# cvlab-stonybrook/s-volsdf

Measured on AMD Instinct MI355X. Metric: rendered rays/sec (1024-ray batch, 128 samples), higher is better.
Workload: dtype f32 (every product, forward and backward, as three fp16 MFMA products of two-piece fp16 operands with f32 accumulate; activation blocks hold both pieces: float32 accuracy class); 1 GPU; configs[1]: VolOpt.train_step (forward + MVS prior lookup + loss + backward + clip/guard/Adam), train mode, fast=1: 1024 rays/GPU x 128 coarse + 98 composited samples + 2048 eikonal points, 8x256 SDF MLP + 4x256 radiance MLP; mode=train, mlp_precision=fp16x2, launch=eager launches, rays_per_gpu=1024, rays_total=1024

## Files before the change

### s-volsdf_amd/csrc/svs_mlp_bwd.hip

```cpp
#include "svs_mlp_dev.h"
#include "svs_mlp_bwd_args.h"
#include "svs_ticket.h"

namespace svs {
namespace mlp {


__global__ __launch_bounds__(kThreads, 1) void rgb_bwd_kernel(RgbBwdArgs a) {
  extern __shared__ __attribute__((aligned(16))) unsigned char smem[];
  Stream st;
  st.g = a.stream; st.buf = reinterpret_cast<f32x4*>(smem); st.cur = 1;
  const int lane = threadIdx.x & 63, half = lane >> 5, wave = threadIdx.x >> 6;
  const int wtile = blockIdx.x * kWaves + wave;
  const int p = wtile * kTilePts + (lane & 31);
  const bool livep = p < a.P;
  const int pc = livep ? p : a.P - 1;
  const size_t LS = block_stride();
  const float* rb = a.rbuf + (size_t)wtile * kBlockF;
  float* zb = a.zbuf + (size_t)wtile * kBlockF;

  st.prefetch<kW4TF4>();
  float dz[3];
#pragma unroll
  for (int c = 0; c < 3; ++c) {
// ... 277 lines not shown
    for (int d = 16; d >= 1; d >>= 1) bsum += __shfl_xor(bsum, d);
    if (lane == 0) atomicAdd(&out[256], bsum);
  }
  det::pass_turn(ticket, blockIdx.x);
}

struct UnpackArgs {
  const float* dWk;
  const float* dbk;
  int ldw;
  int map;
  int rows, cols, row_off;
  const float* v; const float* g;
  float* grad_v; float* grad_g; float* grad_b;
  const float* row0;
};

__device__ __forceinline__ int kernel_col(int map, int c) {
  if (map == 1) return c < 217 ? c : (c < 249 ? 224 + (c - 217) : 217 + (c - 249));
  if (map == 2) return c < 15 ? 256 + c : c - 15;
  if (map == 3) {
    if (c < 172) return c;
    const int e = c - 172;
    return e < 32 ? 224 + e : (e < 64 ? 192 + (e - 32) : 172 + (e - 64));
  }
  if (map == 4) return c < 27 ? 256 + c : c - 27;
  return c;
}

__device__ __forceinline__ void unpack_row(const UnpackArgs& a, int o, int lane) {
  if (o >= a.rows) return;
  const float fac = (a.map == 1 || a.map == 3) ? 0.70710678118654752f : 1.0f;
  const bool is_row0 = a.row0 && o == 0;
  const int ko = o - a.row_off;
  auto dweff = [&](int c) -> float {
    if (is_row0) return a.row0[c];
    return a.dWk[(size_t)ko * a.ldw + kernel_col(a.map, c)] * fac;
  };
  if (lane == 0 && a.grad_b) a.grad_b[o] = is_row0 ? a.row0[256] : (a.dbk ? a.dbk[ko] : 0.0f);
  if (!a.g) {
    for (int c = lane; c < a.cols; c += 64) a.grad_v[(size_t)o * a.cols + c] = dweff(c);
    return;
  }
  double nn = 0.0, dot = 0.0;
  for (int c = lane; c < a.cols; c += 64) {
    const double vv = (double)a.v[(size_t)o * a.cols + c];
    nn += vv * vv; dot += vv * (double)dweff(c);
  }
  for (int d = 32; d >= 1; d >>= 1) { nn += __shfl_xor(nn, d); dot += __shfl_xor(dot, d); }
  const double nrm = __builtin_sqrt(nn);
  const float gg = a.g[o];
  const float k1 = (float)((double)gg / nrm), k2 = (float)((double)gg * dot / (nrm * nn));
  if (lane == 0) a.grad_g[o] = (float)(dot / nrm);
  for (int c = lane; c < a.cols; c += 64)
    a.grad_v[(size_t)o * a.cols + c] = k1 * dweff(c) - k2 * a.v[(size_t)o * a.cols + c];
}

__global__ __launch_bounds__(256) void unpack_wgrad_kernel(UnpackArgs a) {
  unpack_row(a, blockIdx.x * 4 + (threadIdx.x >> 6), threadIdx.x & 63);
}

constexpr int kMaxUnpackJobs = 24;
struct UnpackMulti {
  UnpackArgs job[kMaxUnpackJobs];
  int first_block[kMaxUnpackJobs + 1];
  int n;
};
__global__ __launch_bounds__(256) void unpack_wgrad_multi_kernel(UnpackMulti m) {
  int j = 0;
  while (j + 1 < m.n && (int)blockIdx.x >= m.first_block[j + 1]) ++j;
  unpack_row(m.job[j], ((int)blockIdx.x - m.first_block[j]) * 4 + (threadIdx.x >> 6), threadIdx.x & 63);
}

}
}

using namespace svs;
using namespace svs::mlp;

namespace {
int tiles_of(int n_points) { return (n_points + kWgPts - 1) / kWgPts * kWaves; }
template <typename K>
int set_lds_b(K kernel, int bytes, const char* who) {
  hipError_t e = hipFuncSetAttribute(reinterpret_cast<const void*>(kernel), hipFuncAttributeMaxDynamicSharedMemorySize, bytes);
  if (e != hipSuccess) { set_error("%s: hipFuncSetAttribute: %s", who, hipGetErrorString(e)); return (int)e; }
  return SVS_OK;
}
}

struct svs_unpack_job {
  const float *dWk, *dbk;
  int ldw, map, rows, cols, row_off;
  const float *weight_v, *weight_g, *row0;
  float *grad_v, *grad_g, *grad_b;
};

extern "C" {

size_t svs_block_bytes(int n_points, int blocks_per_tile) {
  return (size_t)tiles_of(n_points) * blocks_per_tile * (kBlockF + 64) * sizeof(float);
}
size_t svs_rgb_zbuf_bytes(int n_points) { return svs_block_bytes(n_points, 5); }
size_t svs_sdf_ubuf_bytes(int n_points) { return svs_block_bytes(n_points, 9); }
size_t svs_sdf_gbuf_bytes(int n_points) { return svs_block_bytes(n_points, 8); }

int svs_rgb_bwd(int n_points, const float* d_rgb, const float* rgb, const float* rbuf, const float* stream, int precision,
                float* zbuf, float* feat_bar, float* d_normals, float* absmax, void* hip_stream) {
  if (!d_rgb || !rgb || !rbuf || !stream || !zbuf || !feat_bar || !d_normals || n_points <= 0) {
    set_error("svs_rgb_bwd: null/invalid argument"); return SVS_EINVAL;
  }
  RgbBwdArgs a{n_points, d_rgb, rgb, rbuf, reinterpret_cast<const f32x4*>(stream), zbuf, feat_bar, d_normals, absmax};
  if (is_h2(precision)) {
    if (!absmax) { set_error("svs_rgb_bwd: fp16x2 needs absmax"); return SVS_EINVAL; }
    return launch_rgb_bwd_h2(a, precision == kFmtF16x2, (hipStream_t)hip_stream);
  }
  if (precision != kFmtF32) { set_error("svs_rgb_bwd: unknown precision %d", precision); return SVS_EINVAL; }
  static int once = set_lds_b(rgb_bwd_kernel, kLdsBytes, "svs_rgb_bwd");
  if (once) return once;
  rgb_bwd_kernel<<<(n_points + kWgPts - 1) / kWgPts, kThreads, kLdsBytes, (hipStream_t)hip_stream>>>(a);
  return check_launch("svs_rgb_bwd");
}

int svs_sdf_bwd_a(const float* points, int n_points, const float* cam, int cam_stride, const float* dirs, const float* z,
                  int S, int n_rays, const float* d_grad, const unsigned char* clamp_mask, const float* hbuf,
                  const float* gbuf, const float* stream, int precision, float* ubuf, float* a2buf, float* pebuf,
                  float* absmax, void* hip_stream) {
  SdfBwdAArgs a;
  const bool h2 = is_h2(precision);
  if (n_points < 0 || n_rays < 0 || (n_points == 0 && n_rays == 0) || (n_points > 0 && !points) ||
      (n_rays > 0 && !(cam && dirs && z && S > 0)) || !d_grad || !hbuf || (!h2 && !gbuf) || !stream || !ubuf || (!h2 && !a2buf) ||
      !pebuf) {
    set_error("svs_sdf_bwd_a: null/invalid argument"); return SVS_EINVAL;
  }
  a.src.pts = points; a.src.cam = cam; a.src.dirs = dirs; a.src.z = z; a.src.cam_stride = cam_stride;
  a.src.S = S > 0 ? S : 1; a.src.n_ray = n_rays * (S > 0 ? S : 0); a.src.P = a.src.n_ray + n_points;
  a.d_grad = d_grad; a.clamp_mask = clamp_mask; a.hbuf = hbuf; a.gbuf = gbuf;
  a.stream = reinterpret_cast<const f32x4*>(stream); a.ubuf = ubuf; a.a2buf = a2buf; a.pebuf = pebuf;
  a.absmax = absmax;
  if (h2) {
    if (!absmax) { set_error("svs_sdf_bwd_a: fp16x2 needs absmax"); return SVS_EINVAL; }
    return launch_sdf_bwd_a_h2(a, precision == kFmtF16x2, (hipStream_t)hip_stream);
  }
  if (precision != kFmtF32) { set_error("svs_sdf_bwd_a: unknown precision %d", precision); return SVS_EINVAL; }
  static int once = set_lds_b(sdf_bwd_a_kernel, kLdsBytes, "svs_sdf_bwd_a");
  if (once) return once;
  sdf_bwd_a_kernel<<<(a.src.P + kWgPts - 1) / kWgPts, kThreads, kLdsBytes, (hipStream_t)hip_stream>>>(a);
  return check_launch("svs_sdf_bwd_a");
}

int svs_sdf_bwd_b(int n_points, const float* d_sdf, const unsigned char* clamp_mask, const float* feat_bar,
                  int n_feat_points, const float* hbuf, const float* gbuf, const float* a2buf, const float* ubuf,
                  const float* stream, int precision, float* abuf, float* sbar_out, float* absmax, void* hip_stream) {
  const bool h2 = is_h2(precision);
  if (!hbuf || !gbuf || (h2 ? !ubuf : !a2buf) || !stream || !abuf || !sbar_out || n_points <= 0 || n_feat_points % 32) {
    set_error("svs_sdf_bwd_b: null/invalid argument (n_feat_points must be a multiple of 32)"); return SVS_EINVAL;
  }
  SdfBwdBArgs a{n_points, d_sdf, clamp_mask, feat_bar, n_feat_points / 32, hbuf, gbuf, a2buf, ubuf,
                reinterpret_cast<const f32x4*>(stream) + kSdfTrainPassBF4, abuf, sbar_out, absmax,
                gbuf + 7 * (size_t)tiles_of(n_points) * kBlockF, (size_t)kBlockF};
  if (h2) {
    if (!absmax) { set_error("svs_sdf_bwd_b: fp16x2 needs absmax"); return SVS_EINVAL; }
    return launch_sdf_bwd_b_h2(a, precision == kFmtF16x2, (hipStream_t)hip_stream);
  }
  if (precision != kFmtF32) { set_error("svs_sdf_bwd_b: unknown precision %d", precision); return SVS_EINVAL; }
  static int once = set_lds_b(sdf_bwd_b_kernel, kLdsBytes, "svs_sdf_bwd_b");
  if (once) return once;
  sdf_bwd_b_kernel<<<(n_points + kWgPts - 1) / kWgPts, kThreads, kLdsBytes, (hipStream_t)hip_stream>>>(a);
  return check_launch("svs_sdf_bwd_b");
}

int svs_lin8_row0_grad(const float* hbuf, const float* ubuf, const float* sbar, int n_points, int precision, float* out257,
                       void* hip_stream) {
  if (!hbuf || !sbar || !out257 || n_points <= 0) { set_error("svs_lin8_row0_grad: bad argument"); return SVS_EINVAL; }
  if (is_h2(precision)) return launch_lin8_row0_h2(hbuf, ubuf, sbar, n_points, tiles_of(n_points), out257, precision == kFmtF16x2, (hipStream_t)hip_stream);
  if (precision != kFmtF32) { set_error("svs_lin8_row0_grad: unknown precision %d", precision); return SVS_EINVAL; }
  const int n_tiles = (n_points + 31) / 32;
  const int grid = n_tiles < 1024 ? n_tiles : 1024;
  const det::Ticket ticket{det::take_slots(1), 0u, (unsigned)grid};
  lin8_row0_kernel<<<grid, 256, 0, (hipStream_t)hip_stream>>>(hbuf, ubuf, sbar, n_tiles, tiles_of(n_points), n_points, out257, ticket);
  return check_launch("svs_lin8_row0_grad");
}

int svs_unpack_wgrad(const float* dWk, const float* dbk, int ldw, int map, int rows, int cols, int row_off,
                     const float* weight_v, const float* weight_g, const float* row0, float* grad_v, float* grad_g,
                     float* grad_b, void* hip_stream) {
  if (!dWk || !weight_v || !grad_v || rows < 1 || cols < 1 || map < 0 || map > 4 || (weight_g && !grad_g)) {
    set_error("svs_unpack_wgrad: bad argument"); return SVS_EINVAL;
  }
  UnpackArgs a{dWk, dbk, ldw, map, rows, cols, row_off, weight_v, weight_g, grad_v, grad_g, grad_b, row0};
  unpack_wgrad_kernel<<<(rows + 3) / 4, 256, 0, (hipStream_t)hip_stream>>>(a);
  return check_launch("svs_unpack_wgrad");
}

int svs_unpack_wgrad_multi(const svs_unpack_job* jobs, int n_jobs, void* hip_stream) {
  if (!jobs || n_jobs < 1 || n_jobs > kMaxUnpackJobs) { set_error("svs_unpack_wgrad_multi: 1..%d jobs", kMaxUnpackJobs); return SVS_EINVAL; }
  UnpackMulti m;
  m.n = n_jobs;
  int blocks = 0;
  for (int i = 0; i < n_jobs; ++i) {
    const svs_unpack_job& q = jobs[i];
    if (!q.dWk || !q.weight_v || !q.grad_v || q.rows < 1 || q.cols < 1 || q.map < 0 || q.map > 4 || (q.weight_g && !q.grad_g)) {
      set_error("svs_unpack_wgrad_multi: bad job %d", i); return SVS_EINVAL;
    }
    m.job[i] = UnpackArgs{q.dWk, q.dbk, q.ldw, q.map, q.rows, q.cols, q.row_off, q.weight_v, q.weight_g, q.grad_v, q.grad_g, q.grad_b, q.row0};
    m.first_block[i] = blocks;
    blocks += (q.rows + 3) / 4;
  }
  m.first_block[n_jobs] = blocks;
  unpack_wgrad_multi_kernel<<<blocks, 256, 0, (hipStream_t)hip_stream>>>(m);
  return check_launch("svs_unpack_wgrad_multi");
}

}
```

### s-volsdf_amd/csrc/svs_mlp_bwd_h2.hip

```cpp
#include "svs_mlp_h2_dev.h"
#include "svs_mlp_host.h"
#include "svs_mlp_bwd_args.h"
#include "svs_mlp_h2_trunk.h"
#include "svs_mlp_bwd_h2_dev.h"
#include "svs_ticket.h"
#include <cstdlib>

namespace svs {
namespace mlp {

template <bool GP>
struct RgbBwdEpi {
  f32x16 prev;
  TilePieces r;
  float v8[8];
  Pieces2* out;
  float* zblk;
  PointScale* ps;
  int lane;
  __device__ __forceinline__ void b(int tp, int rr) {
    float v = prev[rr] * ps->inv_in;
    v = hi_at(r, rr) > 0.0f ? v : 0.0f;
    pin(v);
    ps->track(v);
    v8[rr & 7] = v * ps->s_out;
    if ((rr & 7) == 7) {
      split8(v8, out->h[2 * tp + (rr >> 3)], out->m[2 * tp + (rr >> 3)]);
      pin(out->h[2 * tp + (rr >> 3)], out->m[2 * tp + (rr >> 3)]);
    }
    if (rr == 9) store_piece(zblk, 2 * tp, lane, out->h[2 * tp], 0);
    if (GP && rr == 11) store_piece(zblk, 2 * tp, lane, out->m[2 * tp], 1);
    if (rr == 15) store_grad<GP>(zblk, 2 * tp + 1, lane, out->h[2 * tp + 1], out->m[2 * tp + 1]);
  }
  __device__ __forceinline__ void all(int tp) {
#pragma unroll
    for (int rr = 0; rr < 16; ++rr) b(tp, rr);
  }
};

template <bool GP>
__device__ __forceinline__ void rgb_bwd_layer_h2(Stream& st, const Pieces2& in, Pieces2& out, const float* rblk, float* zblk,
                                                 float* zrec, PointScale& ps, int lane) {
  RgbBwdEpi<GP> ep;
  ep.out = &out; ep.zblk = zblk; ep.ps = &ps; ep.lane = lane;
  store_record(zrec, lane, ps.s_out, 0.0f);
  TilePieces rnext;
  load_tile_hi(rblk, 0, lane, rnext);
#pragma unroll
  for (int t = 0; t < 8; ++t) {
    const TilePieces rcur = rnext;
    auto rload = [&](int s) {
      if (t == 7) return;
      if (s == 10) rnext.h[0] = load_piece(rblk, 2 * (t + 1), lane);
      if (s == 12) rnext.h[1] = load_piece(rblk, 2 * (t + 1) + 1, lane);
    };
    f32x16 acc;
    if (t == 0) acc = tile_mma_h2_pf<16, kChunkF4>(st, in, lane, NoEpi(), NoEpi(), rload);
    else acc = tile_mma_h2_pf<16, kChunkF4>(st, in, lane, NoEpi(), [&](int s) { ep.b(t - 1, s); }, rload);
    ep.prev = acc; ep.r = rcur;
    constexpr int kSt = GP ? 4 : 2;
    if (t == 0) st.advance_keep<2>();
    else if (t < 7) st.advance_keep<2 + kSt>();
    else st.advance_keep<kSt>();
  }
  ep.all(7);
  ps.next();
}

template <bool GP>
__global__ __launch_bounds__(kThreads, 1) void rgb_bwd_h2_kernel(RgbBwdArgs a) {
  extern __shared__ __attribute__((aligned(16))) unsigned char smem[];
  Stream st;
  st.g = a.stream; st.buf = reinterpret_cast<f32x4*>(smem); st.cur = 1;
  const int lane = threadIdx.x & 63, half = lane >> 5, wave = threadIdx.x >> 6;
  const int wtile = blockIdx.x * kWaves + wave;
  const int p = wtile * kTilePts + (lane & 31);
  const bool livep = p < a.P;
  const int pc = livep ? p : a.P - 1;
  const size_t LS = block_stride();
  const float* rb = a.rbuf + (size_t)wtile * kBlockF;
  float* zb = a.zbuf + (size_t)wtile * kBlockF;
  const size_t T = (size_t)gridDim.x * kWaves;
  auto zrec = [&](int l) { return record_ptr(a.zbuf, 5, T, l, wtile); };

  st.prefetch<kW4TF4>();
  float dz[3];
  float m0 = 0.0f;
#pragma unroll
  for (int c = 0; c < 3; ++c) {
    const float o = a.rgb[3 * pc + c];
    dz[c] = (livep && half == 0) ? a.d_rgb[3 * pc + c] * o * (1.0f - o) : 0.0f;
    m0 = __builtin_fmaxf(m0, __builtin_fabsf(dz[c]));
  }
  m0 = __builtin_fmaxf(m0, __shfl_xor(m0, 32));
  PointScale ps;
  ps.start(m0, 0.0f);
  {
    float v8[8] = {dz[0] * ps.s_in, dz[1] * ps.s_in, dz[2] * ps.s_in, 0.0f, 0.0f, 0.0f, 0.0f, 0.0f};
    store_grad8<GP>(zb + 4 * LS, 0, lane, v8);
    store_record(zrec(4), lane, ps.s_in, m0);
  }
  st.advance();
  Pieces2 pa, pb;
  st.prefetch<kChunkF4>();
  {
    const f32x4* c = st.cur_buf();
    const float* r4 = rb + 3 * LS;
    float* z3 = zb + 3 * LS;
    store_record(zrec(3), lane, ps.s_out, 0.0f);
#pragma unroll
    for (int t = 0; t < 8; ++t) {
      TilePieces r;
      load_tile_hi(r4, t, lane, r);
      const f32x4 w = c[t * 64 + lane];
      f32x16 acc = (f32x16)(0.0f);
      acc = __builtin_amdgcn_mfma_f32_32x32x2f32(w[0], dz[0], acc, 0, 0, 0);
      acc = __builtin_amdgcn_mfma_f32_32x32x2f32(w[1], dz[1], acc, 0, 0, 0);
      acc = __builtin_amdgcn_mfma_f32_32x32x2f32(w[2], dz[2], acc, 0, 0, 0);
#pragma unroll
      for (int i = 0; i < 16; ++i) { acc[i] = hi_at(r, i) > 0.0f ? acc[i] : 0.0f; ps.track(acc[i]); }
      split_tile_scaled(acc, t, pa, ps.s_out);
      store_grad<GP>(z3, 2 * t, lane, pa.h[2 * t], pa.m[2 * t]);
      store_grad<GP>(z3, 2 * t + 1, lane, pa.h[2 * t + 1], pa.m[2 * t + 1]);
    }
  }
  ps.next();
  st.advance();
  rgb_bwd_layer_h2<GP>(st, pa, pb, rb + 2 * LS, zb + 2 * LS, zrec(2), ps, lane);
  rgb_bwd_layer_h2<GP>(st, pb, pa, rb + 1 * LS, zb + 1 * LS, zrec(1), ps, lane);
  rgb_bwd_layer_h2<GP>(st, pa, pb, rb, zb, zrec(0), ps, lane);
  float* fb = a.feat_bar + (size_t)wtile * kBlockF;
  float fmax = 0.0f;
  const float s_f = ps.s_out;
  {
    f32x16 prev;
    float v8[8];
    auto slice = [&](int tp, int r) {
      const float v = prev[r] * ps.inv_in;
      fmax = __builtin_fmaxf(fmax, __builtin_fabsf(v));
      v8[r & 7] = v * s_f;
      if ((r & 7) == 7) store_grad8<GP>(fb, 2 * tp + (r >> 3), lane, v8);
    };
#pragma unroll
    for (int t = 0; t < 9; ++t) {
      if (t < 8) st.prefetch<kChunkF4>();
      f32x16 acc;
      if (t == 0) acc = tile_mma_h2<16>(st.cur_buf(), pb, lane);
      else acc = tile_mma_h2<16>(st.cur_buf(), pb, lane, NoEpi(), [&](int s) { slice(t - 1, s); });
      if (t < 8) { prev = acc; st.advance(); }
      else if (half == 1 && livep) {
        a.d_normals[3 * p] = acc[4] * ps.inv_in; a.d_normals[3 * p + 1] = acc[5] * ps.inv_in;
        a.d_normals[3 * p + 2] = acc[6] * ps.inv_in;
      }
    }
  }
  fmax = __builtin_fmaxf(fmax, __shfl_xor(fmax, 32));
  store_record(record_ptr(a.feat_bar, 1, T, 0, wtile), lane, s_f, fmax);
  publish_max(a.absmax + 1, ps.gmax);
  publish_max(a.absmax + 2, fmax);
}

constexpr int kSpliceF = 20;

template <bool SPLIT, bool GP>
struct PassAEpi {
  f32x16 prev;
  TilePieces h;
  float v, s1;
  float v8[8];
  f16x8 up[2], uq[2];
  Pieces2* out;
  float* ublk;
  float* urec;
  PointScale* ps;
  const float* splice;
  float vm;
  int lane, half;
  bool l3;

  __device__ __forceinline__ void begin() {
    if (lane < 32) urec[lane] = ps->s_out;
    vm = 0.0f;
  }
  __device__ __forceinline__ void end() {
    vm = __builtin_fmaxf(vm, __shfl_xor(vm, 32));
    if (lane >= 32) urec[lane] = vm;
  }
  __device__ __forceinline__ void a(int r) {
    v = prev[r] * ps->inv_in;
    s1 = 1.0f - __builtin_amdgcn_exp2f(grad_times<GP>(h, r, -100.0f * 1.44269504088896341f));
    pin(v); pin(s1);
  }
  template <bool LATE = false>
  __device__ __forceinline__ void b(int tp, int r) {
    float u = v * s1;
    float w = __builtin_fabsf(v) * (100.0f - 100.0f * s1);
    if (tp == 6 && r >= 12 && l3) {
      const bool sp = half == 1 || r >= 13;
      const float us = splice[(16 + (r - 12)) * kThreads];
      u = sp ? us : u;
      w = sp ? 0.0f : w;
    }
    pin(u); pin(w);
    emit<LATE>(tp, r, u, w);
  }
  template <bool LATE = false>
  __device__ __forceinline__ void emit(int tp, int r, float u, float w) {
    vm = __builtin_fmaxf(vm, w);
    ps->track(u);
    v8[r & 7] = u * ps->s_out;
    if ((r & 7) == 7) {
      const int k = 2 * tp + (r >> 3), q = r >> 3;
      if (SPLIT) {
        split8(v8, out->h[k], out->m[k]);
        pin(out->h[k], out->m[k]);
        up[q] = out->h[k];
        if (GP) uq[q] = out->m[k];
      } else if (GP) {
        split8(v8, up[q], uq[q]);
      } else {
        up[q] = hi8(v8, 1.0f);
      }
      if (!LATE) store_grad<GP>(ublk, k, lane, up[q], uq[q]);
    }
  }
  __device__ __forceinline__ void store_slot(int tp, int s) {
    if (s == 9) store_piece(ublk, 2 * tp, lane, up[0], 0);
    if (GP && s == 11) store_piece(ublk, 2 * tp, lane, uq[0], 1);
    if (s == 15) store_grad<GP>(ublk, 2 * tp + 1, lane, up[1], uq[1]);
  }
  __device__ __forceinline__ void all(int tp) {
#pragma unroll
    for (int r = 0; r < 16; ++r) { a(r); b(tp, r); }
  }
  __device__ __forceinline__ void splice_tile7() {
#pragma unroll
    for (int r = 0; r < 16; ++r) emit(7, r, splice[r * kThreads], 0.0f);
  }
};

template <bool SPLIT, bool LAST, bool GP>
__device__ __forceinline__ void pass_a_layer_h2(Stream& st, const Pieces2& in, PassAEpi<SPLIT, GP>& ep, const float* hblk, int lane) {
  ep.begin();
#pragma unroll
  for (int t = 0; t < 8; ++t) {
    if (t == 7 && ep.l3) break;
    TilePieces hload;
    load_tile_grad<GP>(hblk, t, lane, hload);
    const bool fetch = !(LAST && t == 7);
    f32x16 acc;
    if (!fetch) acc = tile_mma_h2<16>(st.cur_buf(), in, lane, [&](int s) { ep.a(s); }, [&](int s) { ep.b(t - 1, s); });
    else if (t == 0) acc = tile_mma_h2_pf<16, kChunkF4>(st, in, lane, NoEpi(), NoEpi());
    else acc = tile_mma_h2_pf<16, kChunkF4>(st, in, lane, [&](int s) { ep.a(s); },
                                            [&](int s) { ep.template b<true>(t - 1, s); ep.store_slot(t - 1, s); });
    ep.prev = acc; ep.h = hload;
    if (fetch) {
      if (t == 0) st.advance();
      else st.advance_keep<GP ? 4 : 2>();
    }
  }
  if (ep.l3) { ep.all(6); ep.splice_tile7(); }
  else ep.all(7);
  ep.end();
  ep.ps->next();
}

template <bool GP>
__global__ __launch_bounds__(kThreads, 1) void sdf_bwd_a_h2_kernel(SdfBwdAArgs a) {
  extern __shared__ __attribute__((aligned(16))) unsigned char smem[];
  Stream st;
  st.g = a.stream; st.buf = reinterpret_cast<f32x4*>(smem); st.cur = 1;
  float* splice = reinterpret_cast<float*>(smem + kLdsBytes) + threadIdx.x;
  const int lane = threadIdx.x & 63, half = lane >> 5, wave = threadIdx.x >> 6;
  const int wtile = blockIdx.x * kWaves + wave;
  const int p = wtile * kTilePts + (lane & 31);
  const int pc = p < a.src.P ? p : a.src.P - 1;

  st.prefetch<kChunk0F4>();
  PointScale ps;
  Pieces2 pa, pb;
  const size_t LS = block_stride();
  const float* hb = a.hbuf + (size_t)wtile * kBlockF;
  float* ub = a.ubuf + (size_t)wtile * kBlockF;
  const size_t T = (size_t)gridDim.x * kWaves;
  auto urec = [&](int l) { return record_ptr(a.ubuf, 9, T, l, wtile); };
  {
    float x0, x1, x2;
    load_point(a.src, p, x0, x1, x2);
    PosEnc pe;
    pe.compute(x0, x1, x2);
    float nb[3] = {a.d_grad[3 * pc], a.d_grad[3 * pc + 1], a.d_grad[3 * pc + 2]};
    if (p >= a.src.P || (a.clamp_mask && a.clamp_mask[pc])) { nb[0] = nb[1] = nb[2] = 0.0f; }
    PosEnc u0;
    float m0 = 0.0f;
#pragma unroll
    for (int q = 0; q < 40; ++q) {
      float coef = 1.0f; int c = q;
      if (q >= 3 && q < kPeDim) {
        const int f = (q - 3) / 6, w = (q - 3) % 6;
        const float sc = (float)(1 << f);
        c = w < 3 ? w : w - 3;
        coef = w < 3 ? sc * pe.v[q + 3] : -sc * pe.v[q - 3];
      }
// ... 365 lines not shown
```

### s-volsdf_amd/csrc/svs_mlp_h2.hip

```cpp
#include "svs_mlp_h2_dev.h"
#include "svs_mlp_host.h"
#include "svs_mlp_args.h"
#include "svs_mlp_h2_trunk.h"
#include "svs_blocks_h2.h"

namespace svs {
namespace mlp {

__global__ __launch_bounds__(kThreads, 1) void sdf_only_h2_kernel(SdfOnlyArgs a) {
  extern __shared__ __attribute__((aligned(16))) unsigned char smem[];
  if (a.gate && a.gate[(size_t)(blockIdx.x * kWgPts / a.gate_points) * a.gate_stride] == 0) return;
  Stream st;
  st.g = a.stream;
  st.buf = reinterpret_cast<f32x4*>(smem);
  st.cur = 1;
  const int lane = threadIdx.x & 63, half = lane >> 5, wave = threadIdx.x >> 6;
  const int p = (blockIdx.x * kWaves + wave) * kTilePts + (lane & 31);

  st.prefetch<kChunk0F4>();
  float x0, x1, x2;
  load_point(a.src, p, x0, x1, x2);
  const float r2 = x0 * x0 + x1 * x1 + x2 * x2;
  PosEnc pe;
  pe.compute(x0, x1, x2);
// ... 160 lines not shown
        store_grad<GP>(gb + 7 * block_stride(), 2 * t + 1, lane, xn.h[2 * t + 1], xn.m[2 * t + 1]);
      }
    }
    if (GBUF) store_record(grec0 + 7 * rec_stride, lane, 1.0f, __builtin_fmaxf(gm7, __shfl_xor(gm7, 32)));
    st.advance();
  }
  float* ft = a.feat_tiles ? a.feat_tiles + (size_t)wtile * kBlockF : nullptr;
  {
    f32x16 prev;
    float v8[8];
    f16x8 fh[2], fm[2];
    auto slice = [&](int tp, int r) {
      v8[r & 7] = prev[r];
      if ((r & 7) == 7) { split8(v8, fh[r >> 3], fm[r >> 3]); pin(fh[r >> 3], fm[r >> 3]); }
      if (!ft) return;
      if (r == 9) store_piece(ft, 2 * tp, lane, fh[0], 0);
      if (r == 11) store_piece(ft, 2 * tp, lane, fm[0], 1);
      if (r == 15) { store_piece(ft, 2 * tp + 1, lane, fh[1], 0); store_piece(ft, 2 * tp + 1, lane, fm[1], 1); }
    };
#pragma unroll
    for (int t = 0; t < 8; ++t) {
      f32x16 acc;
      if (t == 0) acc = tile_mma_h2_pf<16, kChunkF4>(st, x, lane, NoEpi(), NoEpi());
      else acc = tile_mma_h2_pf<16, kChunkF4>(st, x, lane, NoEpi(), [&](int s) { slice(t - 1, s); });
      prev = acc;
      if (ft && t > 0) st.advance_keep<4>();
      else st.advance();
    }
#pragma unroll
    for (int r = 0; r < 16; ++r) slice(7, r);
  }
  f32x16 skip7 = (f32x16)(0.0f);
  f32x16 skip6 = (f32x16)(0.0f);
  for (int l = 7; l >= 1; l -= 2) {
    reverse_layer_h2<GBUF, GP>(st, xn, x, l, hb, gb, grec0, rec_stride, skip6, skip7, lane, half);
    if (l > 1) reverse_layer_h2<GBUF, GP>(st, x, xn, l - 1, hb, gb, grec0, rec_stride, skip6, skip7, lane, half);
  }
  st.prefetch<kChunkF4>();
  f32x16 gpe0 = tile_mma_h2<16>(st.cur_buf(), x, lane);
  st.advance();
  f32x16 gpe1 = tile_mma_h2<16>(st.cur_buf(), x, lane);
  gpe0 += skip7;
  gpe1 += skip6;

  if (!GBUF) {
    int p2 = p;
    asm volatile("" : "+v"(p2));
    load_point(a.src, p2, x0, x1, x2);
    pe.compute(x0, x1, x2);
  }
  float dx0 = 0.0f, dx1 = 0.0f, dx2 = 0.0f;
  auto accum = [&](int q, float g, bool active) {
    if (q < 0 || q >= kPeDim) return;
    float coef = 1.0f;
    int c = q;
    if (q >= 3) {
      const int f = (q - 3) / 6, w = (q - 3) % 6;
      const float sc = (float)(1 << f);
      c = w < 3 ? w : w - 3;
      coef = w < 3 ? sc * pe.v[q + 3] : -sc * pe.v[q - 3];
    }
    const float term = active ? coef * g : 0.0f;
    if (c == 0) dx0 += term; else if (c == 1) dx1 += term; else dx2 += term;
  };
#pragma unroll
  for (int r = 0; r < 16; ++r) {
    accum(rho(r), gpe0[r], half == 0);
    accum(rho(r) + 4, gpe0[r], half == 1);
    accum(rho(r) >= 25 ? 32 + rho(r) - 25 : -1, gpe1[r], half == 0);
    accum(rho(r) + 4 >= 25 ? 32 + rho(r) + 4 - 25 : -1, gpe1[r], half == 1);
  }
  dx0 += __shfl_xor(dx0, 32); dx1 += __shfl_xor(dx1, 32); dx2 += __shfl_xor(dx2, 32);

  bool clamped = false;
  if (a.sphere_radius > 0.0f && p < a.clamp_n) {
    const float nrm = __builtin_sqrtf(x0 * x0 + x1 * x1 + x2 * x2);
    const float sphere = a.sphere_scale * (a.sphere_radius - nrm);
    if (sphere < sdf) {
      sdf = sphere;
      const float k = -a.sphere_scale / nrm;
      dx0 = k * x0; dx1 = k * x1; dx2 = k * x2;
      clamped = true;
    }
  }
  if (half == 0 && p < a.src.P && a.clamp_mask) a.clamp_mask[p] = clamped ? 1 : 0;
  if (half == 0 && p < a.src.P) {
    a.sdf[p] = sdf;
    a.grad[3 * p + 0] = dx0; a.grad[3 * p + 1] = dx1; a.grad[3 * p + 2] = dx2;
  }
}

template <bool GP>
struct RgbEpi {
  f32x16 prev;
  float v8[8];
  Pieces2* out;
  float* rblk;
  int lane;
  __device__ __forceinline__ void b(int tp, int r) {
    float v;
    asm("v_max_f32 %0, 0, %1" : "=v"(v) : "v"(prev[r]));
    pin(v);
    v8[r & 7] = v;
    if ((r & 7) == 7) {
      split8(v8, out->h[2 * tp + (r >> 3)], out->m[2 * tp + (r >> 3)]);
      pin(out->h[2 * tp + (r >> 3)], out->m[2 * tp + (r >> 3)]);
    }
    if (rblk) {
      if (r == 11) store_piece(rblk, 2 * tp, lane, out->h[2 * tp], 0);
      if (GP && r == 13) store_piece(rblk, 2 * tp, lane, out->m[2 * tp], 1);
      if (r == 15) store_grad<GP>(rblk, 2 * tp + 1, lane, out->h[2 * tp + 1], out->m[2 * tp + 1]);
    }
  }
  __device__ __forceinline__ void all(int tp) {
#pragma unroll
    for (int r = 0; r < 16; ++r) b(tp, r);
  }
};

template <int KS, int N16NEXT_LAST, bool GP>
__device__ __forceinline__ void rgb_layer_h2(RgbStream& st, const Pieces2& in, Pieces2& out, float* rblk, int lane) {
  RgbEpi<GP> ep;
  ep.out = &out; ep.rblk = rblk; ep.lane = lane;
  constexpr int kNext = KS == 17 ? kRgbChunk0F4 : kChunkF4;
#pragma unroll
  for (int t = 0; t < 8; ++t) {
    auto relu = [&](int s) { if (s < 16) ep.b(t - 1, s); };
    f32x16 acc;
    if (t == 0) acc = tile_mma_h2_pf<KS, kNext>(st, in, lane, NoEpi(), NoEpi());
    else if (t < 7) acc = tile_mma_h2_pf<KS, kNext>(st, in, lane, NoEpi(), relu);
    else acc = tile_mma_h2_pf<KS, N16NEXT_LAST>(st, in, lane, NoEpi(), relu);
    ep.prev = acc;
    if (rblk && t > 0) st.template advance_keep<GP ? 4 : 2>();
    else st.advance();
  }
  ep.all(7);
}

template <bool GP>
__global__ __launch_bounds__(kThreads, 1) void rgb_h2_kernel(RgbArgs a) {
  extern __shared__ __attribute__((aligned(16))) unsigned char smem[];
  RgbStream st;
  st.g = a.stream; st.buf = reinterpret_cast<f32x4*>(smem); st.cur = 1;
  const int lane = threadIdx.x & 63, half = lane >> 5, wave = threadIdx.x >> 6;
  const int wtile = blockIdx.x * kWaves + wave;
  const int p = wtile * kTilePts + (lane & 31);
  const int pc = p < a.src.P ? p : a.src.P - 1;

  st.prefetch<kRgbChunk0F4>();
  float x0, x1, x2;
  load_point(a.src, p, x0, x1, x2);
  const float* vd = a.view + 3 * (size_t)(a.view_S > 0 ? pc / a.view_S : pc);
  const float d0 = vd[0], d1 = vd[1], d2 = vd[2];
  float ex[16];
  ex[0] = x0; ex[1] = x1; ex[2] = x2; ex[3] = d0; ex[4] = d1; ex[5] = d2;
  ex[6] = sinf(d0); ex[7] = sinf(d1); ex[8] = sinf(d2); ex[9] = cosf(d0); ex[10] = cosf(d1); ex[11] = cosf(d2);
  ex[12] = a.normals[3 * pc]; ex[13] = a.normals[3 * pc + 1]; ex[14] = a.normals[3 * pc + 2]; ex[15] = 0.0f;
  float eb[8];
#pragma unroll
  for (int r = 0; r < 8; ++r) eb[r] = half ? ex[rho(r) + 4] : ex[rho(r)];

  Pieces2 x, xn;
  split8(eb, x.h[16], x.m[16]);
  {
    const float* ft = a.feat_tiles + (size_t)wtile * kBlockF;
#pragma unroll
    for (int k = 0; k < 16; ++k) { x.h[k] = load_piece(ft, k, lane, 0); x.m[k] = load_piece(ft, k, lane, 1); }
  }
  const size_t LS = block_stride();
  float* rb = a.rbuf ? a.rbuf + (size_t)wtile * kBlockF : nullptr;
  if (rb) {
    f32x4* d = reinterpret_cast<f32x4*>(a.rbuf + 4 * LS + (size_t)wtile * 1024) + lane;
    f32x4 v0, v1; v0[0] = eb[0]; v0[1] = eb[1]; v0[2] = eb[2]; v0[3] = eb[3]; v1[0] = eb[4]; v1[1] = eb[5]; v1[2] = eb[6]; v1[3] = eb[7];
    d[0] = v0; d[64] = v1; d[128] = (f32x4)(0.0f); d[192] = (f32x4)(0.0f);
  }
  st.advance();

  rgb_layer_h2<17, kChunkF4, GP>(st, x, xn, rb, lane);
  rgb_layer_h2<16, kChunkF4, GP>(st, xn, x, rb ? rb + 1 * LS : nullptr, lane);
  rgb_layer_h2<16, kChunkF4, GP>(st, x, xn, rb ? rb + 2 * LS : nullptr, lane);
  rgb_layer_h2<16, kChunkF4, GP>(st, xn, x, rb ? rb + 3 * LS : nullptr, lane);
  const f32x16 acc = tile_mma_h2<16>(st.cur_buf(), x, lane);
  if (half == 0 && p < a.src.P) {
#pragma unroll
    for (int c = 0; c < 3; ++c) a.rgb[3 * p + c] = 1.0f / (1.0f + __expf(-acc[c]));
  }
}

}
}

using namespace svs;
using namespace svs::mlp;

namespace svs {
namespace mlp {
int launch_sdf_only_h2(const SdfOnlyArgs& a, hipStream_t s) {
  static int once = set_lds(sdf_only_h2_kernel, kLdsBytes, "svs_sdf_vals");
  if (once) return once;
  sdf_only_h2_kernel<<<(a.src.P + kWgPts - 1) / kWgPts, kThreads, kLdsBytes, s>>>(a);
  return check_launch("svs_sdf_vals");
}
int launch_sdf_full_h2(const SdfFullArgs& a, bool grad_pair, hipStream_t s) {
  static int once = set_lds(sdf_full_h2_kernel<true, true>, kLdsBytes, "svs_sdf_outputs") |
                    set_lds(sdf_full_h2_kernel<true, false>, kLdsBytes, "svs_sdf_outputs") |
                    set_lds(sdf_full_h2_kernel<false, false>, kLdsBytes, "svs_sdf_outputs");
  if (once) return once;
  const int grid = (a.src.P + kWgPts - 1) / kWgPts;
  if (!a.gbuf) sdf_full_h2_kernel<false, false><<<grid, kThreads, kLdsBytes, s>>>(a);
  else if (grad_pair) sdf_full_h2_kernel<true, true><<<grid, kThreads, kLdsBytes, s>>>(a);
  else sdf_full_h2_kernel<true, false><<<grid, kThreads, kLdsBytes, s>>>(a);
  return check_launch("svs_sdf_outputs");
}
int launch_rgb_h2(const RgbArgs& a, bool grad_pair, hipStream_t s) {
  constexpr int lds = 2 * kRgbBufF4 * 16;
  static int once = set_lds(rgb_h2_kernel<true>, lds, "svs_rgb_eval") | set_lds(rgb_h2_kernel<false>, lds, "svs_rgb_eval");
  if (once) return once;
  const int grid = (a.src.P + kWgPts - 1) / kWgPts;
  if (grad_pair && a.rbuf) rgb_h2_kernel<true><<<grid, kThreads, lds, s>>>(a);
  else rgb_h2_kernel<false><<<grid, kThreads, lds, s>>>(a);
  return check_launch("svs_rgb_eval");
}
}
}
```

### s-volsdf_amd/svs_hip/train.py

```python
import ctypes
import os

import torch

from . import lib as _lib
from .ops import _f32, _ptr, _ptr_array, _stream, default_precision, is_h2, F16X2, F16X2_HALF

KBLOCK = 128 * 64
KREC = 64


def block_stride(n_points):
    return ((n_points + 127) // 128) * 4 * KBLOCK
LDW = 288


def n_tiles_padded(n_points):
    return ((n_points + 127) // 128) * 4


def record_off(n_points, n_blocks, block):
    T = n_tiles_padded(n_points)
    return n_blocks * T * KBLOCK + block * T * KREC

# ... 38 lines not shown

    def bases(self):
        return self.dWk.data_ptr(), self.dbk.data_ptr(), self.absmax.data_ptr()


class _JobCache(dict):

    def memo(self, key, build):
        hit = self.get(key)
        if hit is None:
            if len(self) >= 64:
                self.clear()
            hit = self[key] = build()
        return hit


def _job_array(jobs):
    arr = (_lib.WGradJob * len(jobs))(*[_lib.WGradJob(*j) for j in jobs])
    return ctypes.cast(arr, ctypes.c_void_p), len(jobs), arr


def _f(addr, n_floats):
    return addr + 4 * n_floats


def wgrad_job(acc, slot, n_pts, amax, scaled, a0, sa0, b0, sb0, a1=None, sa1=0, b1=None, sb1=0, extra=None, sx=0,
              rec0=None, rec1=None):
    dWk, dbk, absmax = acc
    return (a0, b0, sa0, sb0, a1, b1, sa1, sb1, extra, sx, n_pts, LDW, _f(dWk, slot * 256 * LDW), _f(dbk, slot * 256),
            _f(absmax, amax) if scaled else None, rec0 if scaled else None, rec1 if scaled else None)


def rgb_wgrad_table(n_main, h2, acc, zbuf, feat, rbuf):
    LSm = block_stride(n_main)
    zrec = lambda l: _f(zbuf, record_off(n_main, 5, l))
    jobs = [wgrad_job(acc, 9, n_main, 1, h2, zbuf, KBLOCK, feat, KBLOCK, extra=_f(rbuf, 4 * LSm), sx=1024, rec0=zrec(0))]
    for l in range(1, 5):
        jobs.append(wgrad_job(acc, 9 + l, n_main, 1, h2, _f(zbuf, l * LSm), KBLOCK, _f(rbuf, (l - 1) * LSm), KBLOCK,
                              rec0=zrec(l)))
    return jobs


def sdf_wgrad_table(n_total, n_main, h2, acc, abuf, ubuf, pebuf, hbuf, gbuf, feat_bar):
    LS = block_stride(n_total)
    arec = lambda l: _f(abuf, record_off(n_total, 8, l))
    second = lambda l: dict(a1=_f(gbuf, l * LS), sa1=KBLOCK, b1=_f(ubuf, l * LS), sb1=KBLOCK,
                            rec1=_f(ubuf, record_off(n_total, 9, l)))
    jobs = [wgrad_job(acc, 0, n_total, 0, h2, abuf, KBLOCK, pebuf, KBLOCK, rec0=arec(0), **second(0))]
    for l in range(1, 8):
        jobs.append(wgrad_job(acc, l, n_total, 0, h2, _f(abuf, l * LS), KBLOCK, _f(hbuf, (l - 1) * LS), KBLOCK, rec0=arec(l),
                              **second(l)))
    jobs.append(wgrad_job(acc, 8, n_main, 2, h2, feat_bar, KBLOCK, _f(hbuf, 7 * LS), KBLOCK,
                          rec0=_f(feat_bar, record_off(n_main, 1, 0))))
    return jobs


BGRBUF = KBLOCK + 1024


def bg_wgrad_table(P, acc, abuf, zbuf, feat_bar, hbuf, pebuf, rbuf, feat):
    LS, Z2, T = block_stride(P), 2 * KBLOCK, n_tiles_padded(P)
    job = lambda slot, amax, *a, **k: wgrad_job(acc, slot, P, amax, True, *a, **k)
    arec = lambda l: _f(abuf, record_off(P, 8, l))
    jobs = [job(0, 0, abuf, KBLOCK, pebuf, KBLOCK, rec0=arec(0))]
    for l in range(1, 8):
        jobs.append(job(l, 0, _f(abuf, l * LS), KBLOCK, _f(hbuf, (l - 1) * LS), KBLOCK, rec0=arec(l)))
    jobs.append(job(8, 2, feat_bar, KBLOCK, _f(hbuf, 7 * LS), KBLOCK, rec0=_f(feat_bar, record_off(P, 1, 0))))
    zrec = lambda b: _f(zbuf, 2 * T * KBLOCK + b * T * KREC)
    jobs.append(job(9, 1, zbuf, Z2, feat, KBLOCK, rec0=zrec(0), extra=_f(rbuf, KBLOCK), sx=BGRBUF))
    jobs.append(job(10, 1, _f(zbuf, KBLOCK), Z2, rbuf, BGRBUF, rec0=zrec(1)))
    return jobs


def unpack_table(dWk, dbk, row0, layers, maps):
    jobs = []
    for net, l, slot, rows, cols, v, g, gv, gg, gb in layers:
        mp = maps[0] if (net == 0 and l == 4) else (maps[1] if (net == 1 and l == 0) else 0)
        last = net == 0 and l == 8
        jobs.append((_f(dWk, slot * 256 * LDW), _f(dbk, slot * 256), LDW, mp, rows, cols, 1 if last else 0, v, g,
                     row0 if last else None, gv, gg, gb))
    return jobs


def _unpack(accum, nets, maps, out, which=(0, 1)):
    dev = accum.dWk.device
    res, layers, keep = [], [], []
    for gi, (v, g, base) in enumerate(nets):
        group = []
        for l in range(len(v)) if gi in which else ():
            rows, cols = v[l].shape
            if out is not None:
                gv, gg, gb = out[gi][l]
            else:
                gv = torch.empty(rows, cols, device=dev)
                gg = torch.empty(rows, 1, device=dev) if g is not None else None
                gb = torch.empty(rows, device=dev)
            vl, gl = _f32(v[l]), (_f32(g[l]) if g is not None else None)
            keep += [vl, gl]
            layers.append((gi, l, base + l, rows, cols, _ptr(vl), _ptr(gl), _ptr(gv), _ptr(gg), _ptr(gb)))
            group.append((gv, gg, gb))
        res.append(group)
    jobs = unpack_table(_ptr(accum.dWk), _ptr(accum.dbk), _ptr(accum.row0), layers, maps)
    arr = (_lib.UnpackJob * len(jobs))(*[_lib.UnpackJob(*j) for j in jobs])
    _lib.check(_lib.load().svs_unpack_wgrad_multi(ctypes.cast(arr, ctypes.c_void_p), len(jobs), _stream()),
               "svs_unpack_wgrad_multi")
    return res


def finalize(accum, sdf_params, rgb_params, out=None, nets=(0, 1)):
    (sv, sg, _), (rv, rg, _) = sdf_params, rgb_params
    return tuple(_unpack(accum, ((sv, sg, 0), (rv, rg, 9)), (1, 2), out, nets))


class MlpBackward:

    def __init__(self, device, streams=None, accum=None):
        self.dev = device
        self.streams = streams or TrainStreams(device)
        self.accum = accum or WGradAccum(device)
        self._n = None
        self._side = None
        self._job_cache = _JobCache()
        self.time_wgrad = False
        self.timer_events = None

    def _alloc(self, n_total, n_main):
        if self._n == (n_total, n_main):
            return
        L = _lib.load()
        z = lambda nbytes: torch.zeros(nbytes // 4, device=self.dev)
        self.zbuf = z(L.svs_rgb_zbuf_bytes(n_main))
        self.feat_bar = z(L.svs_block_bytes(n_main, 1))
        self.ubuf = z(L.svs_sdf_ubuf_bytes(n_total))
        self.a2buf = z(L.svs_block_bytes(n_total, 8)) if not is_h2(self.streams.precision) else None
        self.abuf = z(L.svs_block_bytes(n_total, 8))
        self.pebuf = z(L.svs_block_bytes(n_total, 1))
        self.sbar = z(L.svs_block_bytes(n_total, 1) // (128 * 2))
        self.d_sdf_full = torch.zeros(n_total, device=self.dev)
        self.d_grad_full = torch.zeros(n_total, 3, device=self.dev)
        self._n = (n_total, n_main)

    def sdf_grad_out(self, n_total, n_main):
        self._alloc(n_total, n_main)
        return self.d_sdf_full[:n_main].view(n_main, 1)

    def grad_extra_out(self, n_total, n_main):
        self._alloc(n_total, n_main)
        return self.d_grad_full[n_main:]

    def accumulate(self, keep, d_rgb, d_sdf, d_grad_extra, wait=True, side=True, defer_wgrad=False, extra=None):
        L = _lib.load()
        src = keep["src"]
        n_total, n_main = src.n, keep["rgb"].shape[0]
        if n_main % 32:
            raise NotImplementedError("rays*samples of a group must be a multiple of 32")
        self._alloc(n_total, n_main)
        dev, acc, S = self.dev, self.accum, self.streams
        hbuf, gbuf, mask = keep["hbuf"], keep["gbuf"], keep["clamp_mask"]
        rbuf, feat = keep["rbuf"], keep["feat_tiles"]

        prec = S.precision
        h2 = is_h2(prec)

        cache, bases = self._job_cache, acc.bases()

        def wgrad_multi(key, build, more):
            own = cache.memo(key, build)
            arr, n, _ = cache.memo(("arr",) + key + ((more["key"],) if more else ()),
                                   lambda: _job_array(own + (more["jobs"] if more else [])))
            _lib.check(L.svs_wgrad_multi(arr, n, prec, _stream()), "svs_wgrad_multi")

        d_rgb = _f32(d_rgb)
        d_grad = self.d_grad_full
        d_normals = d_grad[:n_main]
        n_extra = 0 if d_grad_extra is None else d_grad_extra.shape[0]
        if n_main + n_extra != n_total:
            raise ValueError("d_grad_extra must cover the points that follow the ray samples")
        if n_extra and d_grad_extra.data_ptr() != d_grad[n_main:].data_ptr():
            torch.mul(_f32(d_grad_extra), 1.0, out=d_grad[n_main:])
        _lib.check(L.svs_rgb_bwd(n_main, _ptr(d_rgb), _ptr(keep["rgb"]), _ptr(rbuf), _ptr(S.rgb), prec, _ptr(self.zbuf),
                                 _ptr(self.feat_bar), _ptr(d_normals), _ptr(acc.absmax) if h2 else None, _stream()),
                   "svs_rgb_bwd")
        if d_sdf is not None and d_sdf.data_ptr() == self.d_sdf_full.data_ptr() and d_sdf.numel() == n_main:
            d_sdf_full = self.d_sdf_full
        else:
            d_sdf_full = torch.zeros(n_total, device=dev)
            if d_sdf is not None:
                d_sdf_full[:n_main] = _f32(d_sdf).reshape(-1)
        main = torch.cuda.current_stream()
        if self._side is None:
            self._side = torch.cuda.Stream(device=dev)
        if os.environ.get("SVS_RGB_WGRAD_SIDE", "1") == "0":
            side = False
        side_stream = self._side if side else main
        rkey = ("rgb", n_main, prec, self.zbuf.data_ptr(), feat.data_ptr(), rbuf.data_ptr(), bases[0])
        rgb_jobs = lambda: rgb_wgrad_table(n_main, h2, bases, _ptr(self.zbuf), _ptr(feat), _ptr(rbuf))
        deferred = None
        if defer_wgrad:
            ev_rgb = torch.cuda.Event(); ev_rgb.record(main)
            deferred = dict(rgb=dict(jobs=cache.memo(rkey, rgb_jobs), key=rkey), ev_rgb=ev_rgb)
            join = None
        else:
            fork = torch.cuda.Event(); fork.record(main)
            with torch.cuda.stream(side_stream):
                if side:
                    side_stream.wait_event(fork)
                if extra is not None:
                    side_stream.wait_event(extra["ev_rgb"])
                wgrad_multi(rkey, rgb_jobs, extra["rgb"] if extra else None)
                join = torch.cuda.Event(); join.record(side_stream)
        st = _stream()
        _lib.check(L.svs_sdf_bwd_a(*src.args(), _ptr(d_grad), _ptr(mask), _ptr(hbuf), _ptr(gbuf), _ptr(S.sdf), prec,
                                   _ptr(self.ubuf), _ptr(self.a2buf), _ptr(self.pebuf),
                                   _ptr(acc.absmax) if h2 else None, st), "svs_sdf_bwd_a")
        _lib.check(L.svs_sdf_bwd_b(n_total, _ptr(d_sdf_full), _ptr(mask), _ptr(self.feat_bar), n_main, _ptr(hbuf),
                                   _ptr(gbuf), _ptr(self.a2buf), _ptr(self.ubuf), _ptr(S.sdf), prec, _ptr(self.abuf),
                                   _ptr(self.sbar), _ptr(acc.absmax) if h2 else None, st),
                   "svs_sdf_bwd_b")
        _lib.check(L.svs_lin8_row0_grad(_ptr(hbuf), _ptr(self.ubuf), _ptr(self.sbar), n_total, prec, _ptr(acc.row0),
                                        _stream()), "svs_lin8_row0_grad")
        ev = self.timer_events = ([torch.cuda.Event(enable_timing=True) for _ in range(2)] if self.time_wgrad else None)
        if ev:
            ev[0].record()
        skey = ("sdf", n_total, n_main, prec, self.abuf.data_ptr(), self.ubuf.data_ptr(), self.pebuf.data_ptr(),
                hbuf.data_ptr(), gbuf.data_ptr(), self.feat_bar.data_ptr(), bases[0])
        sdf_jobs = lambda: sdf_wgrad_table(n_total, n_main, h2, bases, _ptr(self.abuf), _ptr(self.ubuf), _ptr(self.pebuf),
                                           _ptr(hbuf), _ptr(gbuf), _ptr(self.feat_bar))
        if defer_wgrad:
            deferred["sdf"] = dict(jobs=cache.memo(skey, sdf_jobs), key=skey)
            deferred["ev_all"] = torch.cuda.Event(); deferred["ev_all"].record(main)
            deferred["hold"] = self._hold = (d_grad, d_sdf_full, d_normals, d_rgb)
            return deferred
        if extra is not None:
            main.wait_event(extra["ev_all"])
        wgrad_multi(skey, sdf_jobs, extra["sdf"] if extra else None)
        if ev:
            ev[1].record()
        if wait and side:
            main.wait_event(join)
        self._hold = (d_grad, d_sdf_full, d_normals, d_rgb)
        return join

    def run(self, sdf_params, rgb_params, keep, d_rgb, d_sdf, d_grad_extra, out=None):
        self.streams.pack(sdf_params, rgb_params)
        self.accum.zero()
        self.accumulate(keep, d_rgb, d_sdf, d_grad_extra)
        return finalize(self.accum, sdf_params, rgb_params, out)


class BgBackward:
    def __init__(self, device, precision=None):
        L = _lib.load()
        self.dev = device
        self.precision = default_precision() if precision is None else int(precision)
        self.sdf_stream = torch.empty(L.svs_stream_bytes(6) // 4, device=device)
        self.rgb_stream = torch.empty(L.svs_stream_bytes(8) // 4, device=device)
        self.ws = torch.empty(L.svs_pack_workspace_bytes() // 4, device=device)
        self.accum = WGradAccum(device, slots=11)
        self.dWk, self.dbk, self.row0, self.absmax = self.accum.dWk, self.accum.dbk, self.accum.row0, self.accum.absmax
        self._job_cache = _JobCache()
        self._scratch = {}

    def pack(self, sdf_wb, rgb_wb):
        L = _lib.load()
        self._keep = []
        for which, (w, b), stream in ((6, sdf_wb, self.sdf_stream), (8, rgb_wb, self.rgb_stream)):
            w, b = [_f32(t) for t in w], [_f32(t) for t in b]
            self._keep += [w, b]
            _lib.check(L.svs_pack_stream(which, self.precision, _ptr_array(w), None, _ptr_array(b), _ptr(self.ws), _ptr(stream),
                                         _stream()), "svs_pack_stream(bg backward)")

    def zero(self):
        self.accum.zero()

    def _alloc(self, n, slot):
        cur = self._scratch.get(slot)
        if cur is not None and cur[0] == n:
            return cur[1:]
        L = _lib.load()
        z = lambda nbytes: torch.zeros(nbytes // 4, device=self.dev)
        cur = (n, z(L.svs_block_bytes(n, 2)),
               z(L.svs_block_bytes(n, 1)), z(L.svs_block_bytes(n, 8)), z(L.svs_block_bytes(n, 1) // (128 * 2)))
        self._scratch[slot] = cur
        return cur[1:]

    def accumulate(self, keep, d_bg_rgb, d_bg_out0, slot=0):
        L = _lib.load()
        P = keep["bg_rgb"].shape[0]
        zbuf, feat_bar, abuf, sbar = self._alloc(P, slot)
        st = _stream()
        hbuf, ghat7, pebuf, rbuf, feat = keep["bg_hbuf"], keep["bg_ghat7"], keep["bg_pebuf"], keep["bg_rbuf"], keep["bg_feat"]
        d_bg_rgb, d_bg_out0 = _f32(d_bg_rgb), _f32(d_bg_out0)
        prec = self.precision
        _lib.check(L.svs_bg_rgb_bwd(P, _ptr(d_bg_rgb), _ptr(keep["bg_rgb"]), _ptr(rbuf), _ptr(self.rgb_stream), prec, _ptr(zbuf),
                                    _ptr(feat_bar), _ptr(self.absmax), st), "svs_bg_rgb_bwd")
        _lib.check(L.svs_bg_sdf_bwd(P, _ptr(d_bg_out0), _ptr(feat_bar), _ptr(hbuf), _ptr(ghat7), _ptr(self.sdf_stream), prec,
                                    _ptr(abuf), _ptr(sbar), _ptr(self.absmax), st), "svs_bg_sdf_bwd")
        _lib.check(L.svs_lin8_row0_grad(_ptr(hbuf), None, _ptr(sbar), P, prec, _ptr(self.row0), st), "svs_lin8_row0_grad")
        ptrs = tuple(_ptr(t) for t in (abuf, zbuf, feat_bar, hbuf, pebuf, rbuf, feat))
        bases = self.accum.bases()
        arr, n, _ = self._job_cache.memo(("bg", P, prec) + ptrs + bases[:1],
                                         lambda: _job_array(bg_wgrad_table(P, bases, *ptrs)))
        _lib.check(L.svs_wgrad_multi(arr, n, prec, st), "svs_wgrad_multi(bg)")
        self._hold = getattr(self, "_hold", {})
        self._hold[slot] = (d_bg_rgb, d_bg_out0)

    def finalize(self, sdf_wb, rgb_wb, out=None):
        if out is not None:
# ... 21 lines not shown
```

Before: 298,200 rays/s.

## Software-pipeline weight prefetch and tile loads in rgb forward/backward kernels

Reworks the radiance MLP backward kernel so weight-chunk prefetches are spread across the MFMA steps (prefetch_step / tile_mma_h2_pf) and uses advance_keep with explicit outstanding-load counts instead of full waits. The next activation tile is loaded one iteration ahead, and the feature-gradient stores are split into piece stores interleaved with compute. The forward rgb kernel issues the feature-tile loads before the sin/cos input encoding so their latency overlaps it. It also relaxes the multiple-of-32 restriction on feature points. Precise wait counts risk reading stale data if they are wrong.

```diff
diff --git a/s-volsdf_amd/csrc/svs_mlp_bwd.hip b/s-volsdf_amd/csrc/svs_mlp_bwd.hip
--- a/s-volsdf_amd/csrc/svs_mlp_bwd.hip
+++ b/s-volsdf_amd/csrc/svs_mlp_bwd.hip
@@ -453,10 +453,11 @@
                   int n_feat_points, const float* hbuf, const float* gbuf, const float* a2buf, const float* ubuf,
                   const float* stream, int precision, float* abuf, float* sbar_out, float* absmax, void* hip_stream) {
   const bool h2 = is_h2(precision);
-  if (!hbuf || !gbuf || (h2 ? !ubuf : !a2buf) || !stream || !abuf || !sbar_out || n_points <= 0 || n_feat_points % 32) {
-    set_error("svs_sdf_bwd_b: null/invalid argument (n_feat_points must be a multiple of 32)"); return SVS_EINVAL;
-  }
-  SdfBwdBArgs a{n_points, d_sdf, clamp_mask, feat_bar, n_feat_points / 32, hbuf, gbuf, a2buf, ubuf,
+  if (!hbuf || !gbuf || (h2 ? !ubuf : !a2buf) || !stream || !abuf || !sbar_out || n_points <= 0 || n_feat_points < 0 ||
+      n_feat_points > n_points) {
+    set_error("svs_sdf_bwd_b: null/invalid argument"); return SVS_EINVAL;
+  }
+  SdfBwdBArgs a{n_points, d_sdf, clamp_mask, feat_bar, (n_feat_points + 31) / 32, hbuf, gbuf, a2buf, ubuf,
                 reinterpret_cast<const f32x4*>(stream) + kSdfTrainPassBF4, abuf, sbar_out, absmax,
                 gbuf + 7 * (size_t)tiles_of(n_points) * kBlockF, (size_t)kBlockF};
   if (h2) {
diff --git a/s-volsdf_amd/csrc/svs_mlp_bwd_h2.hip b/s-volsdf_amd/csrc/svs_mlp_bwd_h2.hip
--- a/s-volsdf_amd/csrc/svs_mlp_bwd_h2.hip
+++ b/s-volsdf_amd/csrc/svs_mlp_bwd_h2.hip
@@ -95,23 +95,26 @@
   m0 = __builtin_fmaxf(m0, __shfl_xor(m0, 32));
   PointScale ps;
   ps.start(m0, 0.0f);
+  const float* r4 = rb + 3 * LS;
+  TilePieces rnext;
+  load_tile_hi(r4, 0, lane, rnext);
   {
     float v8[8] = {dz[0] * ps.s_in, dz[1] * ps.s_in, dz[2] * ps.s_in, 0.0f, 0.0f, 0.0f, 0.0f, 0.0f};
     store_grad8<GP>(zb + 4 * LS, 0, lane, v8);
     store_record(zrec(4), lane, ps.s_in, m0);
   }
-  st.advance();
+  st.advance_keep<2 + (GP ? 3 : 2)>();
   Pieces2 pa, pb;
-  st.prefetch<kChunkF4>();
   {
     const f32x4* c = st.cur_buf();
-    const float* r4 = rb + 3 * LS;
     float* z3 = zb + 3 * LS;
     store_record(zrec(3), lane, ps.s_out, 0.0f);
 #pragma unroll
     for (int t = 0; t < 8; ++t) {
-      TilePieces r;
-      load_tile_hi(r4, t, lane, r);
+      TilePieces r = rnext;
+      pin(r.h[0], r.h[1]);
+      st.prefetch_step<kChunkF4, 8>(t);
+      if (t < 7) load_tile_hi(r4, t + 1, lane, rnext);
       const f32x4 w = c[t * 64 + lane];
       f32x16 acc = (f32x16)(0.0f);
       acc = __builtin_amdgcn_mfma_f32_32x32x2f32(w[0], dz[0], acc, 0, 0, 0);
@@ -123,9 +126,10 @@
       store_grad<GP>(z3, 2 * t, lane, pa.h[2 * t], pa.m[2 * t]);
       store_grad<GP>(z3, 2 * t + 1, lane, pa.h[2 * t + 1], pa.m[2 * t + 1]);
     }
+    st.prefetch_done<kChunkF4>();
   }
   ps.next();
-  st.advance();
+  st.advance_keep<GP ? 8 : 4>();
   rgb_bwd_layer_h2<GP>(st, pa, pb, rb + 2 * LS, zb + 2 * LS, zrec(2), ps, lane);
   rgb_bwd_layer_h2<GP>(st, pb, pa, rb + 1 * LS, zb + 1 * LS, zrec(1), ps, lane);
   rgb_bwd_layer_h2<GP>(st, pa, pb, rb, zb, zrec(0), ps, lane);
@@ -135,20 +139,37 @@
   {
     f32x16 prev;
     float v8[8];
+    f16x8 fh[2], fm[2];
     auto slice = [&](int tp, int r) {
       const float v = prev[r] * ps.inv_in;
       fmax = __builtin_fmaxf(fmax, __builtin_fabsf(v));
       v8[r & 7] = v * s_f;
-      if ((r & 7) == 7) store_grad8<GP>(fb, 2 * tp + (r >> 3), lane, v8);
+      if ((r & 7) == 7) {
+        const int q = r >> 3;
+        if (GP) {
+          split8(v8, fh[q], fm[q]);
+          pin(fh[q], fm[q]);
+        } else {
+#pragma unroll
+          for (int j = 0; j < 8; ++j) fh[q][j] = (_Float16)v8[j];
+          fm[q] = fh[q];
+        }
+      }
+      if (r == 9) store_piece(fb, 2 * tp, lane, fh[0], 0);
+      if (GP && r == 11) store_piece(fb, 2 * tp, lane, fm[0], 1);
+      if (r == 15) store_grad<GP>(fb, 2 * tp + 1, lane, fh[1], fm[1]);
     };
+    constexpr int kSt = GP ? 4 : 2;
 #pragma unroll
     for (int t = 0; t < 9; ++t) {
-      if (t < 8) st.prefetch<kChunkF4>();
       f32x16 acc;
-      if (t == 0) acc = tile_mma_h2<16>(st.cur_buf(), pb, lane);
-      else acc = tile_mma_h2<16>(st.cur_buf(), pb, lane, NoEpi(), [&](int s) { slice(t - 1, s); });
-      if (t < 8) { prev = acc; st.advance(); }
-      else if (half == 1 && livep) {
+      if (t == 0) acc = tile_mma_h2_pf<16, kChunkF4>(st, pb, lane, NoEpi(), NoEpi());
+      else if (t < 8) acc = tile_mma_h2_pf<16, kChunkF4>(st, pb, lane, NoEpi(), [&](int s) { slice(t - 1, s); });
+      else acc = tile_mma_h2<16>(st.cur_buf(), pb, lane, NoEpi(), [&](int s) { slice(7, s); });
+      if (t < 8) {
+        prev = acc;
+        if (t == 0) st.advance(); else st.advance_keep<kSt>();
+      } else if (half == 1 && livep) {
         a.d_normals[3 * p] = acc[4] * ps.inv_in; a.d_normals[3 * p + 1] = acc[5] * ps.inv_in;
         a.d_normals[3 * p + 2] = acc[6] * ps.inv_in;
       }
diff --git a/s-volsdf_amd/csrc/svs_mlp_h2.hip b/s-volsdf_amd/csrc/svs_mlp_h2.hip
--- a/s-volsdf_amd/csrc/svs_mlp_h2.hip
+++ b/s-volsdf_amd/csrc/svs_mlp_h2.hip
@@ -336,29 +336,34 @@
   load_point(a.src, p, x0, x1, x2);
   const float* vd = a.view + 3 * (size_t)(a.view_S > 0 ? pc / a.view_S : pc);
   const float d0 = vd[0], d1 = vd[1], d2 = vd[2];
+  const float n0 = a.normals[3 * pc], n1 = a.normals[3 * pc + 1], n2 = a.normals[3 * pc + 2];
+  Pieces2 x, xn;
+  {
+    const float* ft = a.feat_tiles + (size_t)wtile * kBlockF;
+#pragma unroll
+    for (int k = 0; k < 16; ++k) {
+      x.h[k] = load_piece(ft, k, lane, 0); x.m[k] = load_piece(ft, k, lane, 1);
+      asm volatile("" ::: "memory");
+    }
+  }
   float ex[16];
   ex[0] = x0; ex[1] = x1; ex[2] = x2; ex[3] = d0; ex[4] = d1; ex[5] = d2;
   ex[6] = sinf(d0); ex[7] = sinf(d1); ex[8] = sinf(d2); ex[9] = cosf(d0); ex[10] = cosf(d1); ex[11] = cosf(d2);
-  ex[12] = a.normals[3 * pc]; ex[13] = a.normals[3 * pc + 1]; ex[14] = a.normals[3 * pc + 2]; ex[15] = 0.0f;
+  ex[12] = n0; ex[13] = n1; ex[14] = n2; ex[15] = 0.0f;
   float eb[8];
 #pragma unroll
   for (int r = 0; r < 8; ++r) eb[r] = half ? ex[rho(r) + 4] : ex[rho(r)];
-
-  Pieces2 x, xn;
   split8(eb, x.h[16], x.m[16]);
-  {
-    const float* ft = a.feat_tiles + (size_t)wtile * kBlockF;
-#pragma unroll
-    for (int k = 0; k < 16; ++k) { x.h[k] = load_piece(ft, k, lane, 0); x.m[k] = load_piece(ft, k, lane, 1); }
-  }
   const size_t LS = block_stride();
   float* rb = a.rbuf ? a.rbuf + (size_t)wtile * kBlockF : nullptr;
   if (rb) {
     f32x4* d = reinterpret_cast<f32x4*>(a.rbuf + 4 * LS + (size_t)wtile * 1024) + lane;
     f32x4 v0, v1; v0[0] = eb[0]; v0[1] = eb[1]; v0[2] = eb[2]; v0[3] = eb[3]; v1[0] = eb[4]; v1[1] = eb[5]; v1[2] = eb[6]; v1[3] = eb[7];
     d[0] = v0; d[64] = v1; d[128] = (f32x4)(0.0f); d[192] = (f32x4)(0.0f);
-  }
-  st.advance();
+    st.advance_keep<32 + 4>();
+  } else {
+    st.advance_keep<32>();
+  }
 
   rgb_layer_h2<17, kChunkF4, GP>(st, x, xn, rb, lane);
   rgb_layer_h2<16, kChunkF4, GP>(st, xn, x, rb ? rb + 1 * LS : nullptr, lane);
diff --git a/s-volsdf_amd/svs_hip/train.py b/s-volsdf_amd/svs_hip/train.py
--- a/s-volsdf_amd/svs_hip/train.py
+++ b/s-volsdf_amd/svs_hip/train.py
@@ -214,8 +214,6 @@
         L = _lib.load()
         src = keep["src"]
         n_total, n_main = src.n, keep["rgb"].shape[0]
-        if n_main % 32:
-            raise NotImplementedError("rays*samples of a group must be a multiple of 32")
         self._alloc(n_total, n_main)
         dev, acc, S = self.dev, self.accum, self.streams
         hbuf, gbuf, mask = keep["hbuf"], keep["gbuf"], keep["clamp_mask"]
```

Measured after the change: 299,600 rays/s (median of 4 runs). No clear change (+0.5%).
